# jzbontar/mc-cnn

Measured on AMD Instinct MI355X. Metric: Mega-pixel-disparities/sec (cost-vol+CBCA+SGM) + end-to-end disp ms/pair, higher is better.
Workload: dtype f32; 1 GPU; KITTI 2012 fast, 370x1226 disp_max=228; H=370, W=1226, disp_max=228, feature_channels=64, params=kitti_fast, parallelism=one pair per GPU

## Files before the change

mc-cnn_amd/csrc/post.hip:

```cpp
#include "launchers.h"

#include <atomic>

namespace mc {


__global__ void __launch_bounds__(256) fill_nan_kernel(float *__restrict__ p, int64_t n)
{
	const float nanv = __builtin_nanf("");
	for (int64_t i = (int64_t)blockIdx.x * blockDim.x + threadIdx.x; i < n; i += (int64_t)gridDim.x * blockDim.x) p[i] = nanv;
}

__global__ void __launch_bounds__(256) scale_kernel(const float *__restrict__ in, float *__restrict__ out, int64_t n, float s)
{
	for (int64_t i = (int64_t)blockIdx.x * blockDim.x + threadIdx.x; i < n; i += (int64_t)gridDim.x * blockDim.x) out[i] = in[i] * s;
}
typedef float f4v_t __attribute__((ext_vector_type(4)));
__global__ void __launch_bounds__(256) scale4_kernel(const f4v_t *__restrict__ in, f4v_t *__restrict__ out, int64_t n4, float s)
{
	const int64_t i = (int64_t)blockIdx.x * 256 + threadIdx.x;
	if (i < n4) out[i] = in[i] * s;
}

template <bool NT>
// ... 7 lines not shown
		const int64_t r = r0 + k, c = c0 + tx;
		if (r < R && c < Cn) tile[k][tx] = NT ? __builtin_nontemporal_load(in + r * ldin + c) : in[r * ldin + c];
	}
	__syncthreads();
	for (int k = ty; k < 64; k += 4) {
		const int64_t c = c0 + k, r = r0 + tx;
		if (r < R && c < Cn) {
			if (NT) __builtin_nontemporal_store(tile[tx][k] * s, out + c * ldout + r);
			else out[c * ldout + r] = tile[tx][k] * s;
		}
	}
}

typedef float post_f4 __attribute__((ext_vector_type(4)));
template <bool NT, bool LOOP_R>
__global__ void __launch_bounds__(256) transpose4_kernel(const float *__restrict__ in, float *__restrict__ out, int64_t R,
                                                         int64_t Cn, int64_t ldin, int64_t ldout, float s)
{
	__shared__ float tile[64][65];
	const int lx = threadIdx.x & 15, ly = threadIdx.x >> 4;
	const int64_t fixed0 = (int64_t)blockIdx.x * 64;
	const int64_t nloop = LOOP_R ? R : Cn;
	for (int64_t t0 = 0; t0 < nloop; t0 += 64) {
		const int64_t c0 = LOOP_R ? fixed0 : t0, r0 = LOOP_R ? t0 : fixed0;
#pragma unroll
		for (int k = 0; k < 4; ++k) {
			const int row = ly + 16 * k;
			const int64_t r = r0 + row, c = c0 + 4 * lx;
			if (r < R && c < Cn) {
				const post_f4 *p = (const post_f4 *)(in + r * ldin + c);
				const post_f4 v = NT ? __builtin_nontemporal_load(p) : *p;
				tile[row][4 * lx + 0] = v.x; tile[row][4 * lx + 1] = v.y; tile[row][4 * lx + 2] = v.z; tile[row][4 * lx + 3] = v.w;
			}
		}
		__syncthreads();
#pragma unroll
		for (int k = 0; k < 4; ++k) {
			const int col = ly + 16 * k;
			const int64_t c = c0 + col, r = r0 + 4 * lx;
			if (c < Cn && r < R) {
				const post_f4 v = {tile[4 * lx + 0][col] * s, tile[4 * lx + 1][col] * s, tile[4 * lx + 2][col] * s, tile[4 * lx + 3][col] * s};
				post_f4 *q = (post_f4 *)(out + c * ldout + r);
				if (NT) __builtin_nontemporal_store(v, q);
				else *q = v;
			}
		}
		__syncthreads();
	}
}


int fill_nan(float *p, int64_t n, hipStream_t st)
{
	if (n <= 0) return 0;
	const unsigned blocks = cdiv(n, 256) < 4096u ? cdiv(n, 256) : 4096u;
	hipLaunchKernelGGL(fill_nan_kernel, dim3(blocks), dim3(256), 0, st, p, n);
	return check_launch("fill_nan");
}

int scale(const float *in, float *out, int64_t n, float s, hipStream_t st)
{
	if (n <= 0) return 0;
	if (n % 4 == 0 && (uintptr_t)in % 16 == 0 && (uintptr_t)out % 16 == 0 && n / 4 / 256 < 0x7fffffff) {
		hipLaunchKernelGGL(scale4_kernel, dim3(cdiv(n / 4, 256)), dim3(256), 0, st, (const f4v_t *)in, (f4v_t *)out, n / 4, s);
		return check_launch("scale");
	}
	const unsigned blocks = cdiv(n, 256) < 4096u ? cdiv(n, 256) : 4096u;
	hipLaunchKernelGGL(scale_kernel, dim3(blocks), dim3(256), 0, st, in, out, n, s);
	return check_launch("scale");
}

int transpose(const float *in, float *out, int64_t R, int64_t Cn, int64_t ldin, int64_t ldout, float s, hipStream_t st, int nt)
{
	const bool use_nt = nt >= 0 ? nt != 0 : R * Cn * 4 > ((int64_t)768 << 20);
	const bool aligned16 = Cn % 4 == 0 && ldin % 4 == 0 && ldout % 4 == 0 && (uintptr_t)in % 16 == 0 && (uintptr_t)out % 16 == 0;
	if (R % 4 == 0 && aligned16) {
		if (R <= Cn) {
			if (use_nt) hipLaunchKernelGGL((transpose4_kernel<true, true>), dim3(cdiv(Cn, 64)), dim3(256), 0, st, in, out, R, Cn, ldin, ldout, s);
			else hipLaunchKernelGGL((transpose4_kernel<false, true>), dim3(cdiv(Cn, 64)), dim3(256), 0, st, in, out, R, Cn, ldin, ldout, s);
		} else {
			if (use_nt) hipLaunchKernelGGL((transpose4_kernel<true, false>), dim3(cdiv(R, 64)), dim3(256), 0, st, in, out, R, Cn, ldin, ldout, s);
			else hipLaunchKernelGGL((transpose4_kernel<false, false>), dim3(cdiv(R, 64)), dim3(256), 0, st, in, out, R, Cn, ldin, ldout, s);
		}
		return check_launch("transpose");
	}
	if (use_nt) hipLaunchKernelGGL(transpose_kernel<true>, dim3(cdiv(Cn, 64), cdiv(R, 64)), dim3(256), 0, st, in, out, R, Cn, ldin, ldout, s);
	else hipLaunchKernelGGL(transpose_kernel<false>, dim3(cdiv(Cn, 64), cdiv(R, 64)), dim3(256), 0, st, in, out, R, Cn, ldin, ldout, s);
	return check_launch("transpose");
}

__global__ void __launch_bounds__(256) fix_border_kernel(float *__restrict__ vol, int64_t rows, int W, int n, int direction)
{
	const int64_t id = (int64_t)blockIdx.x * blockDim.x + threadIdx.x;
	if (id >= rows * n) return;
	const int i = (int)(id % n) + 1;
	const int64_t r = id / n;
	const int dst = direction < 0 ? W - i : i - 1;
	const int src = direction < 0 ? W - (n + 1) : n;
	vol[r * W + dst] = vol[r * W + src];
}

int fix_border(float *vol, int D, int H, int W, int n, int direction, hipStream_t st)
{
	if (n <= 0) return 0;
	const int64_t rows = (int64_t)D * H;
	hipLaunchKernelGGL(fix_border_kernel, dim3(cdiv(rows * n, 256)), dim3(256), 0, st, vol, rows, W, n, direction);
	return check_launch("fix_border");
}

__global__ void __launch_bounds__(256) argmin_dhw_kernel(const float *__restrict__ vol, float *__restrict__ out, int D, int64_t HW,
                                                         int base1)
{
	const int64_t p = (int64_t)blockIdx.x * blockDim.x + threadIdx.x;
	if (p >= HW) return;
	int argmin = 0;
	float mn = __builtin_inff();
	for (int i = 0; i < D; ++i) {
		const float val = __builtin_nontemporal_load(vol + i * HW + p);
		if (val < mn) {
			mn = val;
			argmin = i;
		}
	}
	out[p] = (float)(argmin + base1);
}

__global__ void __launch_bounds__(256) argmin_dhw4_kernel(const float *__restrict__ vol, float *__restrict__ out, int D, int64_t HW,
                                                          int base1)
{
	const int64_t p = ((int64_t)blockIdx.x * blockDim.x + threadIdx.x) * 4;
	if (p >= HW) return;
	int a0 = 0, a1 = 0, a2 = 0, a3 = 0;
	float m0 = __builtin_inff(), m1 = m0, m2 = m0, m3 = m0;
	for (int i = 0; i < D; ++i) {
		const post_f4 v = __builtin_nontemporal_load((const post_f4 *)(vol + i * HW + p));
		if (v.x < m0) { m0 = v.x; a0 = i; }
		if (v.y < m1) { m1 = v.y; a1 = i; }
		if (v.z < m2) { m2 = v.z; a2 = i; }
		if (v.w < m3) { m3 = v.w; a3 = i; }
	}
	*(post_f4 *)(out + p) = post_f4{(float)(a0 + base1), (float)(a1 + base1), (float)(a2 + base1), (float)(a3 + base1)};
}

int argmin_dhw(const float *vol, float *out, int D, int H, int W, int base1, hipStream_t st)
{
	const int64_t HW = (int64_t)H * W;
	if (HW % 4 == 0 && (uintptr_t)vol % 16 == 0 && (uintptr_t)out % 16 == 0)
		hipLaunchKernelGGL(argmin_dhw4_kernel, dim3(cdiv(HW / 4, 256)), dim3(256), 0, st, vol, out, D, HW, base1);
	else
		hipLaunchKernelGGL(argmin_dhw_kernel, dim3(cdiv(HW, 256)), dim3(256), 0, st, vol, out, D, HW, base1);
	return check_launch("argmin_dhw");
}

__global__ void __launch_bounds__(256) outlier_rows_kernel(const float *__restrict__ d0, const float *__restrict__ d1,
                                                           float *__restrict__ outlier, int W, int disp_max)
{
	extern __shared__ unsigned char mark[];
	const int y = blockIdx.x;
	const int64_t row = (int64_t)y * W;
	for (int x = threadIdx.x; x < W; x += 256) mark[x] = 0;
	__syncthreads();
	for (int xp = threadIdx.x; xp < W; xp += 256) {
		const float v = d1[row + xp];
		if (v > -2.0f && v < (float)disp_max + 2.0f) {
			const int base = (int)floorf(v);
#pragma unroll
			for (int k = -2; k <= 3; ++k) {
				const int d = base + k;
				if (d >= 0 && d < disp_max && xp + d < W && (double)fabsf((float)d - v) < 1.1) mark[xp + d] = 1;
			}
		}
	}
	__syncthreads();
	for (int x = threadIdx.x; x < W; x += 256) {
		const int64_t id = row + x;
		const int d0i = (int)d0[id];
		float res;
		if (x - d0i < 0) res = 1;
		else if ((double)fabsf(d0[id] - d1[id - d0i]) < 1.1) res = 0;
		else res = mark[x] ? 2.0f : 1.0f;
		outlier[id] = res;
	}
}

struct LdsRaised {
	std::atomic<int> cus[64] = {};
	int raise(const void *kernel, int bytes, const char *who, int *ncu = nullptr)
	{
		int dev = 0;
		hipError_t e = hipGetDevice(&dev);
		if (e == hipSuccess && (dev < 0 || dev >= 64)) e = hipErrorInvalidDevice;
		if (e != hipSuccess) {
			set_error("%s: hipGetDevice: %s (device %d)", who, hipGetErrorString(e), dev);
			return (int)e;
		}
		int n = cus[dev].load(std::memory_order_acquire);
		if (!n) {
			e = hipFuncSetAttribute(kernel, hipFuncAttributeMaxDynamicSharedMemorySize, bytes);
			if (e == hipSuccess) e = hipDeviceGetAttribute(&n, hipDeviceAttributeMultiprocessorCount, dev);
			if (e != hipSuccess || n <= 0) {
				set_error("%s: %d bytes of dynamic LDS on device %d: %s", who, bytes, dev, hipGetErrorString(e));
				return e != hipSuccess ? (int)e : MC_EINVAL;
			}
			cus[dev].store(n, std::memory_order_release);
		}
		if (ncu) *ncu = n;
		return 0;
	}
};

int outlier_detection(const float *d0, const float *d1, float *outlier, int H, int W, int disp_max, hipStream_t st)
{
	MC_REQUIRE(W <= 160 * 1024, "outlier_detection: a row of %d pixels needs more than the 160 KiB of LDS its marks live in", W);
	if (W > 64 * 1024) {
		static LdsRaised raised;
		const int rc = raised.raise((const void *)outlier_rows_kernel, 160 * 1024, "outlier_detection");
		if (rc) return rc;
	}
	hipLaunchKernelGGL(outlier_rows_kernel, dim3(H), dim3(256), (size_t)W, st, d0, d1, outlier, W, disp_max);
	return check_launch("outlier_detection");
}

__global__ void __launch_bounds__(256) interp_occ_rows_kernel(const float *__restrict__ d0, const float *__restrict__ outlier,
                                                              float *__restrict__ out, int W, unsigned *__restrict__ mask, int size)
{
	__shared__ int carry[256];
	__shared__ int first_valid;
	const int y = blockIdx.x, t = threadIdx.x;
	const int64_t row = (int64_t)y * W;
	if (mask) {
		const int wa = (int)((row + 31) >> 5), wb = (int)((row + W + 31) >> 5);
		for (int w0 = wa; w0 < wb; w0 += 8) {
			const int p = w0 * 32 + t;
			const uint64_t bal = __ballot(p < size && outlier[p] == 2);
			const int w = w0 + (t >> 5);
			if ((t & 31) == 0 && w < wb) mask[w] = (unsigned)(bal >> (t & 32));
		}
	}
	const int seg = (W + 255) / 256;
	const int xa = t * seg, xb = min(W, xa + seg);
	if (t == 0) first_valid = W;
	int last = -1;
	for (int x = xa; x < xb; ++x)
		if (outlier[row + x] == 0) last = x;
	carry[t] = last;
	__syncthreads();
	if (last >= 0) {
		int f = -1;
		for (int x = xa; x < xb; ++x)
			if (outlier[row + x] == 0) { f = x; break; }
		atomicMin(&first_valid, f);
	}
	for (int off = 1; off < 256; off <<= 1) {
		const int o = t >= off ? carry[t - off] : -1;
		__syncthreads();
		carry[t] = max(carry[t], o);
		__syncthreads();
	}
	int lv = t > 0 ? carry[t - 1] : -1;
	const int fv = first_valid;
	for (int x = xa; x < xb; ++x) {
		const int64_t id = row + x;
		const float o = outlier[id];
		if (o == 0) lv = x;
		float r = d0[id];
		if (o == 1) {
			if (lv >= 0) r = d0[row + lv];
			else if (fv < W) r = d0[row + fv];
		}
		out[id] = r;
	}
}

int interpolate_occlusion(const float *d0, const float *outlier, float *out, int H, int W, hipStream_t st, unsigned *mask)
{
	if (mask) MC_REQUIRE((int64_t)H * W < ((int64_t)1 << 31), "interpolate_occlusion: %dx%d pixels do not fit the mask's 32-bit index", H, W);
	hipLaunchKernelGGL(interp_occ_rows_kernel, dim3(H), dim3(256), 0, st, d0, outlier, out, W, mask, mask ? H * W : 0);
	return check_launch("interpolate_occlusion");
}

template <int K> __device__ __forceinline__ void ray_rank_step(float v, int inb, int &less, int &eq)
{
	const float ov = __uint_as_float(__builtin_amdgcn_update_dpp(0u, __float_as_uint(v), 0x120 + K, 0xf, 0xf, false));
	const int oin = __builtin_amdgcn_update_dpp(0, inb, 0x120 + K, 0xf, 0xf, false);
	less += (oin && ov < v) ? 1 : 0;
	eq += (oin && ov == v) ? 1 : 0;
}

#define MC_MIS_NU 4
constexpr int MIS_NT = 1024;
constexpr unsigned MIS_OOB = 0x80000000u;

__device__ __forceinline__ void ray_select(float v, int inb, int ray, int id, const float *__restrict__ d0, float *__restrict__ out)
{
	int less = 0, eq = inb;
	ray_rank_step<1>(v, inb, less, eq); ray_rank_step<2>(v, inb, less, eq); ray_rank_step<3>(v, inb, less, eq);
	ray_rank_step<4>(v, inb, less, eq); ray_rank_step<5>(v, inb, less, eq); ray_rank_step<6>(v, inb, less, eq);
	ray_rank_step<7>(v, inb, less, eq); ray_rank_step<8>(v, inb, less, eq); ray_rank_step<9>(v, inb, less, eq);
	ray_rank_step<10>(v, inb, less, eq); ray_rank_step<11>(v, inb, less, eq); ray_rank_step<12>(v, inb, less, eq);
	ray_rank_step<13>(v, inb, less, eq); ray_rank_step<14>(v, inb, less, eq); ray_rank_step<15>(v, inb, less, eq);
	const uint64_t bal = __ballot(inb != 0);
	const int n = __builtin_popcount((unsigned)((bal >> ((threadIdx.x & 48))) & 0xffffu));
	if (n == 0) {
		if (ray == 0) out[id] = d0[id];
		return;
	}
	const int want = n / 2;
	if (inb && less <= want && want < less + eq) out[id] = v;
}

__device__ __forceinline__ void mis_rays_masked(const float *__restrict__ d0, const float *__restrict__ outlier, float *__restrict__ out,
                                                int size, int H, int W, const unsigned *__restrict__ mask, int per)
{
	static_assert(MC_MIS_NU == 4, "the round below is two whole-pixel steps");
	extern __shared__ unsigned mis_lds[];
	__shared__ int wave_n[MIS_NT / 64];
	__shared__ int next_item;
	const int nw = (size + 31) >> 5;
	unsigned *lmask = mis_lds;
	unsigned *slot = lmask + nw;
	int *list_y = (int *)(slot + MIS_NT * 16);
	unsigned short *list = (unsigned short *)(list_y + MIS_NT);
	const int tid = threadIdx.x, lane = tid & 63, wid = tid >> 6;
	const int pa = blockIdx.x * per, pb = min(size, pa + per);
	if (pa >= pb) return;
	for (int i = tid; i < nw; i += MIS_NT) lmask[i] = mask[i];
	constexpr unsigned HX_LO = 0x10000012u, HX_HI = 0x34444432u, HY_LO = 0x00123444u, HY_HI = 0x44321000u;
	const unsigned xmax2 = 2u * (unsigned)W - 2u, ymax2 = 2u * (unsigned)H - 2u;
	for (int c0 = pa; c0 < pb; c0 += MIS_NT) {
		const int p = c0 + tid;
		bool mis = false;
		if (p < pb) {
			const float v = d0[p];
			mis = outlier[p] == 2;
			if (!mis) out[p] = v;
		}
		const uint64_t bal = __ballot(mis);
		if (lane == 0) wave_n[wid] = __builtin_popcountll(bal);
		if (tid == 0) next_item = MIS_NT;
		__syncthreads();
		int base = 0, nlist = 0;
#pragma unroll
		for (int k = 0; k < MIS_NT / 64; ++k) {
			const int c = wave_n[k];
			base += k < wid ? c : 0;
			nlist += c;
		}
		if (mis) {
			const int j = base + __builtin_popcountll(bal & (((uint64_t)1 << lane) - 1));
			list[j] = (unsigned short)tid;
			list_y[j] = p / W;
		}
		__syncthreads();
		const int nitems = nlist * 16;
		int i = tid;
		int q = 0, X2 = 0, Y2 = 0, sx = 0, sy = 0, o1 = 0, o2 = 0;
		auto start = [&]() {
			const int j = i >> 4, ray = i & 15, sh = 4 * (ray & 7);
			sx = (int)(((ray < 8 ? HX_LO : HX_HI) >> sh) & 15u) - 2;
			sy = (int)(((ray < 8 ? HY_LO : HY_HI) >> sh) & 15u) - 2;
			q = c0 + list[j];
			const int y = list_y[j];
			X2 = 2 * (q - y * W);
			Y2 = 2 * y;
			o1 = ((sy + 1) >> 1) * W + ((sx + 1) >> 1);
			o2 = sy * W + sx;
		};
		if (i < nitems) start();
		while (i < nitems) {
			const int o[MC_MIS_NU] = {o1, o2, o2 + o1, 2 * o2};
			unsigned off[MC_MIS_NU], m[MC_MIS_NU];
#pragma unroll
			for (int k = 0; k < MC_MIS_NU; ++k) {
				X2 += sx;
				Y2 += sy;
				const bool in = (unsigned)X2 <= xmax2 && (unsigned)Y2 <= ymax2;
				const unsigned a = in ? (unsigned)(q + o[k]) : 0u;
				off[k] = in ? a : MIS_OOB;
				m[k] = lmask[a >> 5] >> (a & 31);
				m[k] = in ? m[k] & 1u : 0u;
			}
			q += 2 * o2;
			unsigned stop = MIS_OOB;
			bool stopped = false;
#pragma unroll
			for (int k = MC_MIS_NU - 1; k >= 0; --k) {
				const bool hit = m[k] == 0;
				stop = hit ? off[k] : stop;
				stopped = hit ? true : stopped;
			}
			if (stopped) {
				slot[i] = stop;
				i = atomicAdd(&next_item, 1);
				if (i < nitems) start();
			}
		}
		__syncthreads();
		const int ray = tid & 15;
		int j = tid >> 4;
		unsigned stop = j < nlist ? slot[j * 16 + ray] : MIS_OOB;
		float v = d0[stop != MIS_OOB ? stop : 0u];
		while (j < nlist) {
			const int jn = j + MIS_NT / 16;
			const unsigned stop_n = jn < nlist ? slot[jn * 16 + ray] : MIS_OOB;
			const float v_n = d0[stop_n != MIS_OOB ? stop_n : 0u];
			ray_select(stop != MIS_OOB ? v : 0.0f, stop != MIS_OOB ? 1 : 0, ray, c0 + list[j], d0, out);
			j = jn;
			stop = stop_n;
			v = v_n;
		}
		__syncthreads();
	}
}

__global__ void __launch_bounds__(MIS_NT) interp_mis_rays_kernel(const float *__restrict__ d0, const float *__restrict__ outlier,
                                                                 float *__restrict__ out, int size, int H, int W,
                                                                 const unsigned *__restrict__ mask, int per)
{
	if (mask) {
		mis_rays_masked(d0, outlier, out, size, H, W, mask, per);
		return;
	}
	const int t = blockIdx.x * blockDim.x + threadIdx.x;
// ... 404 lines not shown
```

mc-cnn_amd/csrc/sgm.hip:

```cpp
#include "launchers.h"

#define MC_SGM_VOL_AUX 2
#define MC_SGM_ST_AUX MC_SGM_VOL_AUX

namespace mc {

constexpr int SGM_PADW = 520;

struct SgmPassArgs {
	const float *C[2];
	const float *accin[2];
	const float *accin2[2];
	float *out[2];
	float *out2[2];
	float *disp[2];
	int drop_out[2];
	int direction[2];
	int nvol;
	int H, W, D, ds;
	int tri;
	const uint8_t *cls0;
	int64_t cls_plane;
	const uint8_t *win;
	int Wm;
	float P1[3], P2[3], P1a[3];
	int drop_h[2];
};

__device__ __forceinline__ int cls_of(float v, float tau) { return v < tau ? 0 : (v > tau ? 2 : 1); }

__global__ void __launch_bounds__(256) sgm_prep_kernel(const float *__restrict__ x0, const float *__restrict__ x1,
                                                       uint8_t *__restrict__ cls0, uint8_t *__restrict__ win,
                                                       int H, int W, int Wm, int64_t cls_plane, float tau_so)
{
	const int64_t id = (int64_t)blockIdx.x * blockDim.x + threadIdx.x;
	const int64_t total = (int64_t)4 * H * Wm;
	if (id >= total) return;
	const int i = (int)(id % Wm);
	const int y = (int)((id / Wm) % H);
	const int r = (int)(id / ((int64_t)Wm * H));
	const int dx = r == 0 ? 1 : (r == 1 ? -1 : 0);
	const int dy = r == 2 ? 1 : (r == 3 ? -1 : 0);
	const bool yok = (y - dy >= 0) && (y - dy < H);

	if (i < W) {
		const int x = i;
		int c = 1;
		if (yok && x - dx >= 0 && x - dx < W) {
			c = cls_of(fabsf(x0[y * W + x] - x0[(y - dy) * W + x - dx]), tau_so);
		}
		cls0[(int64_t)r * cls_plane + (int64_t)y * W + x] = (uint8_t)c;
	}
	const int s = i - SGM_PADW;
	unsigned asc = 0, desc = 0;
#pragma unroll
	for (int k = 0; k < 4; ++k) {
		const int xx = s + k;
		float D2 = 10.0f;
		if (yok && xx >= 0 && xx < W && xx - dx >= 0 && xx - dx < W) {
			D2 = fabsf(x1[y * W + xx] - x1[(y - dy) * W + xx - dx]);
		}
		const unsigned c = (unsigned)cls_of(D2, tau_so);
		asc |= c << (2 * k);
		desc |= c << (2 * (3 - k));
	}
	win[((int64_t)(0 * 4 + r) * H + y) * Wm + i] = (uint8_t)asc;
	win[((int64_t)(1 * 4 + r) * H + y) * Wm + i] = (uint8_t)desc;
}

typedef unsigned uint4v __attribute__((ext_vector_type(4)));

template <int VPL, int NACC>
struct StepData {
	float c[VPL];
	float a[NACC > 0 ? VPL : 1];
	float a2[NACC > 1 ? VPL : 1];
	unsigned pk;
	unsigned a0;
};


__device__ __forceinline__ float vmin2(float a, float b)
{
	float r;
	asm("v_min_f32 %0, %1, %2" : "=v"(r) : "v"(a), "v"(b));
	return r;
}
__device__ __forceinline__ float vmin3(float a, float b, float c)
{
	float r;
	asm("v_min3_f32 %0, %1, %2, %3" : "=v"(r) : "v"(a), "v"(b), "v"(c));
	return r;
}
__device__ __forceinline__ float wave_min_q(float v)
{
	float r;
	asm volatile("s_nop 1\n\tv_min_f32_dpp %1, %1, %1 quad_perm:[1,0,3,2] row_mask:0xf bank_mask:0xf\n\t"
	             "s_nop 1\n\tv_min_f32_dpp %1, %1, %1 quad_perm:[2,3,0,1] row_mask:0xf bank_mask:0xf\n\t"
	             "s_nop 1\n\tv_min_f32_dpp %1, %1, %1 row_half_mirror row_mask:0xf bank_mask:0xf\n\t"
	             "s_nop 1\n\tv_min_f32_dpp %1, %1, %1 row_mirror row_mask:0xf bank_mask:0xf\n\t"
	             "s_nop 1\n\tv_min_f32_dpp %1, %1, %1 row_bcast:15 row_mask:0xa bank_mask:0xf\n\t"
	             "s_nop 1\n\tv_min_f32_dpp %1, %1, %1 row_bcast:31 row_mask:0xc bank_mask:0xf\n\t"
	             "s_nop 0\n\tv_readlane_b32 %0, %1, 63"
	             : "=s"(r), "+v"(v));
	return r;
}

__device__ __forceinline__ __amdgpu_buffer_rsrc_t pixel_rsrc(const float *base, int64_t elem_off, int bytes)
{
	return __builtin_amdgcn_make_buffer_rsrc((void *)(base + elem_off), 0, bytes, 0x00020000);
}

template <int DIRN, int VPL, int MODE, bool ARGMIN, bool VEC, int U, bool DUAL, bool FAR, bool TRIH>
__device__ __forceinline__ void sgm_line(const SgmPassArgs &A, int wave)
{
	static_assert(!TRIH || (DIRN == 0 && DUAL && MODE == 0 && VEC && !FAR && !ARGMIN), "TRIH: the fused horizontal launch only");
	constexpr int NACC = MODE == 0 ? 0 : (MODE == 3 ? 2 : 1);
	const int lane = threadIdx.x & 63;
	const int H = A.H, W = A.W, D = A.D, ds = A.ds, Wm = A.Wm;
	const int nlines = DIRN <= 1 ? H : W;
	const int nsteps = DIRN <= 1 ? W : H;
	const int nw = A.nvol * nlines;
	bool second = false;
	if (DUAL) {
		if (wave >= 2 * nw) return;
		second = wave >= nw;
		if (second) wave -= nw;
	} else if (wave >= nw) {
		return;
	}
	const int dirn = (DUAL && second) ? 1 : DIRN;
	const int v = wave / nlines;
	const int line = wave - v * nlines;
	const int direction = A.direction[v];
	const float *__restrict__ Cp = A.C[v];
	const float *__restrict__ Ain = A.accin[v];
	const float *__restrict__ Ain2 = A.accin2[v];
	float *__restrict__ Out = (DUAL && second) ? A.out2[v] : A.out[v];
	float *__restrict__ Disp = A.disp[v];
	const bool drop = A.drop_out[v];

	const int x0s = dirn == 0 ? 0 : (dirn == 1 ? W - 1 : line);
	const int y0s = dirn == 2 ? 0 : (dirn == 3 ? H - 1 : line);
	const int sx = dirn == 0 ? 1 : (dirn == 1 ? -1 : 0);
	const int sy = dirn == 2 ? 1 : (dirn == 3 ? -1 : 0);

	const int dbase = VPL * lane;
	const uint8_t *__restrict__ cls0 = A.cls0 + (int64_t)dirn * A.cls_plane;
	constexpr int WBIAS = 1024;
	const uint8_t *__restrict__ win = A.win + ((int64_t)((direction > 0 ? 0 : 1) * 4 + dirn) * H) * Wm + SGM_PADW - WBIAS;
	const int woff = (direction > 0 ? dbase : -dbase - 3) + WBIAS;
	const int wq = direction > 0 ? 4 : -4;
	const int run_bytes = (VEC ? ds : D) * 4;
	constexpr bool TRI = DIRN >= 2 && MODE >= 2;
	int Dv = D;
	if (TRI && A.tri) Dv = __builtin_amdgcn_readfirstlane(min(D, direction < 0 ? line + 1 : W - line));
	const unsigned live_bytes = (TRI && Dv < D) ? (unsigned)Dv * 4u : (unsigned)run_bytes;

	const float INF = __builtin_inff();
	const float P1mid = A.P1[1], P2mid = A.P2[1], P1amid = A.P1a[1];
	const float P1lo = A.P1[0], P2lo = A.P2[0], P1alo = A.P1a[0];
	const float P1hi = A.P1[2], P2hi = A.P2[2], P1ahi = A.P1a[2];

	const int last = nsteps - 1;
	const int pix0 = y0s * W + x0s, dp = sy * W + sx;
	const int minpix = dp > 0 ? pix0 : pix0 + last * dp;
	const unsigned c1v = (unsigned)(dp * ds * 4);
	const unsigned c0v = dp > 0 ? 0u : (unsigned)last * (unsigned)(-dp * ds * 4);
	const unsigned span = (unsigned)last * (unsigned)((dp > 0 ? dp : -dp) * ds * 4) + (unsigned)run_bytes;
	constexpr unsigned OOBV = 0x80000000u;
	const __amdgpu_buffer_rsrc_t rC = pixel_rsrc(Cp, (int64_t)minpix * ds, FAR ? 0 : span);
	const __amdgpu_buffer_rsrc_t rA = pixel_rsrc(NACC >= 1 ? Ain : Cp, (int64_t)minpix * ds, FAR ? 0 : span);
	const __amdgpu_buffer_rsrc_t rA2 = pixel_rsrc(NACC >= 2 ? Ain2 : Cp, (int64_t)minpix * ds, FAR ? 0 : span);
	const __amdgpu_buffer_rsrc_t rO = pixel_rsrc(Out, (int64_t)minpix * ds, (FAR || drop) ? 0 : span);
	const __amdgpu_buffer_rsrc_t rW = __builtin_amdgcn_make_buffer_rsrc((void *)win, 0, H * Wm + 2 * WBIAS + 64, 0x00020000);
	const int w0 = y0s * Wm + x0s, dw = sy * Wm + sx;
	const __amdgpu_buffer_rsrc_t rCls = __builtin_amdgcn_make_buffer_rsrc((void *)cls0, 0, H * W, 0x00020000);
	const __amdgpu_buffer_rsrc_t rDisp = pixel_rsrc(ARGMIN ? Disp : Out, 0, H * W * 4);
	unsigned lane_off[VEC ? VPL / 4 : VPL];
#pragma unroll
	for (int q = 0; q < (VEC ? VPL / 4 : VPL); ++q) {
		const unsigned b = (unsigned)(dbase + (VEC ? 4 * q : q)) * 4u;
		lane_off[q] = ((FAR && !TRI) || b < live_bytes) ? b : OOBV;
	}
	const unsigned lane0_off = lane == 0 ? 0u : OOBV;
	const int hdv0 = direction < 0 ? x0s + 1 : W - x0s, hdv1 = direction < 0 ? sx : -sx;
	const bool trim_st = TRIH && (second || A.drop_h[v] != 0);
	const int sdv0 = trim_st ? hdv0 : D, sdv1 = trim_st ? hdv1 : 0;
	auto live_bytes_of = [&](int dv) -> unsigned { return dv < D ? (unsigned)dv * 4u : (unsigned)run_bytes; };
	auto live_at = [&](int s) -> unsigned { return live_bytes_of(hdv0 + s * hdv1); };
	auto piece_off = [&](int q, unsigned lim) -> unsigned {
		const unsigned b = (unsigned)(dbase + 4 * q) * 4u;
		return b < lim ? b : OOBV;
	};

	auto load_run = [&](float (&dst)[VPL], const float *base, const __amdgpu_buffer_rsrc_t &rs, unsigned so, int64_t pix, unsigned lim = 0u) {
		const __amdgpu_buffer_rsrc_t r = FAR ? pixel_rsrc(base, pix * ds, run_bytes) : rs;
		const unsigned soff = FAR ? 0u : so;
		if (VEC) {
#pragma unroll
			for (int q = 0; q < VPL / 4; ++q) {
				const uint4v t = __builtin_amdgcn_raw_buffer_load_b128(r, TRIH ? piece_off(q, lim) : lane_off[q], soff, MC_SGM_VOL_AUX);
				dst[4 * q + 0] = __uint_as_float(t.x); dst[4 * q + 1] = __uint_as_float(t.y);
				dst[4 * q + 2] = __uint_as_float(t.z); dst[4 * q + 3] = __uint_as_float(t.w);
			}
		} else {
#pragma unroll
			for (int j = 0; j < VPL; ++j) dst[j] = __uint_as_float(__builtin_amdgcn_raw_buffer_load_b32(r, lane_off[j], soff, 0));
		}
	};

	auto load_step = [&](StepData<VPL, NACC> &sd, int s) {
		const unsigned so = c0v + (unsigned)s * c1v;
		const int64_t pix = FAR ? (int64_t)(y0s + s * sy) * W + (x0s + s * sx) : 0;
		load_run(sd.c, Cp, rC, so, pix, TRIH ? live_at(s) : 0u);
		if constexpr (NACC >= 1) load_run(sd.a, Ain, rA, so, pix);
		if constexpr (NACC >= 2) load_run(sd.a2, Ain2, rA2, so, pix);
		unsigned pk = 0;
		const unsigned sw = (unsigned)(w0 + s * dw);
#pragma unroll
// ... 58 lines not shown
		}
		const int a0 = __builtin_amdgcn_readfirstlane((int)sd.a0);
		const int amatch = a0 == 1 ? 3 : a0;
		float P1x, P2x, P1ax = 0.0f;
		if (DIRN >= 2)
			asm("s_cmp_eq_u32 %3, 0\n\ts_cselect_b32 %0, %4, %5\n\ts_cselect_b32 %1, %6, %7\n\ts_cselect_b32 %2, %8, %9"
			    : "=s"(P1x), "=s"(P2x), "=s"(P1ax)
			    : "s"(a0), "s"(P1lo), "s"(P1hi), "s"(P2lo), "s"(P2hi), "s"(P1alo), "s"(P1ahi)
			    : "scc");
		else
			asm("s_cmp_eq_u32 %2, 0\n\ts_cselect_b32 %0, %3, %4\n\ts_cselect_b32 %1, %5, %6"
			    : "=s"(P1x), "=s"(P2x)
			    : "s"(a0), "s"(P1lo), "s"(P1hi), "s"(P2lo), "s"(P2hi)
			    : "scc");
		const float down = lane_from_below(prev[VPL - 1], INF);
		const float up = lane_from_above(prev[0], INF);
#pragma unroll
		for (int j = 0; j < VPL; ++j) {
			const int b = (sd.pk >> (2 * j)) & 3;
			const bool match = b == amatch;
			const float P2 = match ? P2x : P2midv;
			const float P1 = match ? P1x : P1midv;
			const float P1a = match ? P1ax : P1amidv;
			const float pm = j > 0 ? prev[j > 0 ? j - 1 : 0] : down;
			const float pp = j < VPL - 1 ? prev[j < VPL - 1 ? j + 1 : 0] : up;
			float cost;
			asm("v_min_f32 %0, %1, %2\n\tv_min3_f32 %0, %0, %3, %4"
			    : "=&v"(cost)
			    : "v"(prev[j]), "v"(m + P2), "v"(pm + (DIRN == 2 ? P1a : P1)), "v"(pp + (DIRN == 3 ? P1a : P1)));
			val[j] = (c[j] + cost) - m;
		}
		if (s == 0) {
			asm volatile("; border step");
#pragma unroll
			for (int j = 0; j < VPL; ++j) val[j] = c[j];
		}
		float q[VPL];
#pragma unroll
		for (int j = 0; j < VPL; ++j) {
			if (MODE == 0) o[j] = val[j] + zadd;
			else if (MODE == 1) o[j] = sd.a[j] + val[j];
			else if (MODE == 2) o[j] = (sd.a[j] + val[j]) * 0.25f;
			else o[j] = (sd.a[j] + sd.a2[j]) + val[j];
			q[j] = vmin2(val[j], INFv);
		}
#pragma unroll
		for (int j = 0; j < VPL; ++j) prev[j] = (dbase + j < Dv) ? q[j] : INFv;
		float nm = vmin3(prev[0], prev[1], prev[2]);
#pragma unroll
		for (int j = 3; j < VPL; j += 2) nm = j + 1 < VPL ? vmin3(nm, prev[j], prev[j + 1]) : vmin2(nm, prev[j]);
		m = wave_min_q(nm);
		if (keep) {
#pragma unroll
			for (int j = 0; j < VPL; ++j) keep[j] = o[j];
		} else {
			store_step(o, s);
		}
	};

	StepData<VPL, NACC> ring[U];
#pragma unroll
	for (int u = 0; u < U; ++u) load_step(ring[u], u < last ? u : last);

	int g = 0;
	constexpr int SB = (DIRN <= 1 && !ARGMIN && U % 4 == 0) ? 4 : 1;
	constexpr int LB = (DIRN <= 1 && U % 4 == 0) ? 4 : 1;
	float obuf[SB][VPL];
	for (; g + U <= nsteps; g += U) {
#pragma unroll
		for (int u = 0; u < U; ++u) {
			const int s = g + u;
			__builtin_amdgcn_sched_barrier(0);
			if (SB > 1) {
				process(ring[u], s, obuf[u % SB]);
				if (u % SB == SB - 1) {
#pragma unroll
					for (int k = 0; k < SB; ++k) store_step(obuf[k], s - (SB - 1) + k);
				}
			} else {
				process(ring[u], s);
			}
			if (u % LB == LB - 1) {
#pragma unroll
				for (int k = 0; k < LB; ++k) {
					const int sn = s - (LB - 1) + k + U;
					load_step(ring[u - (LB - 1) + k], sn < last ? sn : last);
				}
			}
		}
	}
#pragma unroll
	for (int u = 0; u < U; ++u) {
		if (g + u < nsteps) process(ring[u], g + u);
	}
}

template <int DIRN, int VPL, int MODE, bool ARGMIN, bool VEC, int U, bool DUAL, bool FAR>
__global__ void __launch_bounds__(256) sgm_pass_kernel(const SgmPassArgs A)
{
	const int wave = __builtin_amdgcn_readfirstlane((int)((blockIdx.x * blockDim.x + threadIdx.x) >> 6));
	if constexpr (DIRN == 0 && DUAL && MODE == 0 && VEC && !FAR && !ARGMIN) {
		if (A.tri) {
			sgm_line<DIRN, VPL, MODE, ARGMIN, VEC, U, DUAL, FAR, true>(A, wave);
			return;
		}
	}
	sgm_line<DIRN, VPL, MODE, ARGMIN, VEC, U, DUAL, FAR, false>(A, wave);
}


__global__ void __launch_bounds__(256) sgm_contract_kernel(const float *__restrict__ vol, int64_t pixels, int D, unsigned *__restrict__ count)
{
	const int64_t p = (int64_t)blockIdx.x * blockDim.x + threadIdx.x;
	bool bad = false;
	if (p < pixels) {
		const float *v = vol + p * D;
		bad = !(fabsf(v[0]) < __builtin_inff());
		bool seen_nan = false;
		for (int d = 0; d < D; ++d) {
			const bool isn = v[d] != v[d];
			bad = bad || (seen_nan && !isn);
			seen_nan = seen_nan || isn;
		}
	}
	const unsigned long long b = __ballot(bad);
	if ((threadIdx.x & 63) == 0 && b) atomicAdd(count, (unsigned)__builtin_popcountll(b));
}

int sgm_contract_violations(const float *vol, int H, int W, int D, unsigned *count, hipStream_t st)
{
	const int64_t pixels = (int64_t)H * W;
	hipError_t e = hipMemsetAsync(count, 0, sizeof(unsigned), st);
	if (e != hipSuccess) {
		set_error("mc_sgm2_contract_violations: hipMemsetAsync: %s", hipGetErrorString(e));
		return (int)e;
	}
	hipLaunchKernelGGL(sgm_contract_kernel, dim3(cdiv(pixels, 256)), dim3(256), 0, st, vol, pixels, D, count);
	return check_launch("sgm_contract");
}

struct SgmMaps { int Wm; size_t plane, cls0, win, bytes; };
static SgmMaps sgm_maps(int H, int W)
{
	const int Wm = W + 2 * SGM_PADW;
	const size_t plane = ((size_t)H * W + 3 + 4) / 4 * 4;
	return {Wm, plane, 0, 4 * plane, (4 * plane + (size_t)8 * H * Wm + 255) & ~(size_t)255};
}

size_t sgm_maps_bytes(int H, int W) { return sgm_maps(H, W).bytes; }

int sgm_prep(const float *x0, const float *x1, void *maps, int H, int W, float tau_so, hipStream_t st)
{
	const SgmMaps m = sgm_maps(H, W);
	const int64_t total = (int64_t)4 * H * m.Wm;
	hipLaunchKernelGGL(sgm_prep_kernel, dim3(cdiv(total, 256)), dim3(256), 0, st, x0, x1, (uint8_t *)maps + m.cls0, (uint8_t *)maps + m.win, H, W,
	                   m.Wm, (int64_t)m.plane, tau_so);
	return check_launch("sgm_prep");
}

constexpr int SGM_U_H = 8, SGM_U_UP = 16;
constexpr int SGM_U_DOWN = 16;

template <int DIRN, int MODE, bool ARGMIN, bool DUAL>
static void launch_pass(const SgmPassArgs &A, bool vec, hipStream_t st)
{
	const int nlines = DIRN <= 1 ? A.H : A.W;
	const int waves = A.nvol * nlines * (DUAL ? 2 : 1);
	const dim3 grid(cdiv(waves, 4)), block(256);
	const int U = DIRN == 2 ? SGM_U_DOWN : (DIRN == 3 ? SGM_U_UP : SGM_U_H);
	constexpr bool SCALAR = MODE == 1;
#define MC_SGM_GO(VPL_, VEC_, U_) \
	hipLaunchKernelGGL((sgm_pass_kernel<DIRN, VPL_, MODE, ARGMIN, VEC_, U_, DUAL, false>), grid, block, 0, st, A)
#define MC_SGM_GO_FAR(VPL_, VEC_, U_) \
	hipLaunchKernelGGL((sgm_pass_kernel<DIRN, VPL_, MODE, ARGMIN, VEC_, U_, DUAL, true>), grid, block, 0, st, A)
	const bool far = (int64_t)A.H * A.W * A.ds * 4 >= ((int64_t)1 << 31);
	if (!vec) {
		if constexpr (SCALAR) {
			if (far) { if (A.D <= 256) MC_SGM_GO_FAR(4, false, 4); else MC_SGM_GO_FAR(8, false, 2); }
			else { if (A.D <= 256) MC_SGM_GO(4, false, 4); else MC_SGM_GO(8, false, 2); }
		}
	} else if (far) {
		if (A.D <= 256) MC_SGM_GO_FAR(4, true, 4); else MC_SGM_GO_FAR(8, true, 4);
	} else if (A.D <= 256) {
		if (U == 16) MC_SGM_GO(4, true, 16); else if (U == 8) MC_SGM_GO(4, true, 8); else MC_SGM_GO(4, true, 4);
	} else {
		if (U >= 8) MC_SGM_GO(8, true, 8); else MC_SGM_GO(8, true, 4);
	}
#undef MC_SGM_GO_FAR
#undef MC_SGM_GO
}


int sgm_sweeps(const float *const C[2], float *const out[2], float *const out2[2], float *const disp[2],
               const int direction[2], int nvol, int H, int W, int D, int ds, const void *maps, float pi1, float pi2,
               float alpha1, float q1, float q2, bool fused, unsigned drop_final, bool tri, hipStream_t st)
{
	MC_REQUIRE((int64_t)H * W < ((int64_t)1 << 29) && (int64_t)W * ds * 4 < ((int64_t)1 << 31), "sgm: image %dx%d (pixel stride %d) exceeds the sweeps' 32-bit line arithmetic", H, W, ds);
	SgmPassArgs A;
	for (int v = 0; v < 2; ++v) {
		const int k = v < nvol ? v : 0;
		A.C[v] = C[k];
		A.accin[v] = out[k];
		A.accin2[v] = out2 ? out2[k] : nullptr;
		A.out[v] = out[k];
		A.out2[v] = out2 ? out2[k] : nullptr;
		A.disp[v] = disp ? disp[k] : nullptr;
		A.direction[v] = direction[k];
		A.drop_out[v] = 0;
		A.drop_h[v] = (fused && tri && v < nvol && ((drop_final >> v) & 1)) ? 1 : 0;
	}
	A.nvol = nvol;
	A.tri = (fused && tri) ? 1 : 0;
	A.H = H; A.W = W; A.D = D; A.ds = ds;
	const SgmMaps m = sgm_maps(H, W);
	A.Wm = m.Wm;
	A.cls0 = (const uint8_t *)maps + m.cls0;
	A.cls_plane = (int64_t)m.plane;
	A.win = (const uint8_t *)maps + m.win;
	A.P1[0] = pi1; A.P2[0] = pi2;
	A.P1[1] = pi1 / q1; A.P2[1] = pi2 / q1;
	A.P1[2] = pi1 / (q1 * q2); A.P2[2] = pi2 / (q1 * q2);
	for (int k = 0; k < 3; ++k) A.P1a[k] = A.P1[k] / alpha1;

	bool vec = (ds % 4 == 0);
	for (int v = 0; v < nvol; ++v) {
		vec = vec && ((uintptr_t)C[v] % 16 == 0) && ((uintptr_t)out[v] % 16 == 0);
		if (out2) vec = vec && ((uintptr_t)out2[v] % 16 == 0);
	}
	const bool am = fused && disp && disp[0];
	if (!fused) {
		launch_pass<0, 1, false, false>(A, vec, st);
		launch_pass<1, 1, false, false>(A, vec, st);
		launch_pass<2, 1, false, false>(A, vec, st);
		launch_pass<3, 1, false, false>(A, vec, st);
	} else {
		MC_REQUIRE(out2 && vec, "sgm: the fused sweeps need the second direction's scratch and 16-byte aligned volumes with ds %% 4 == 0");
		launch_pass<0, 0, false, true>(A, vec, st);
		launch_pass<2, 3, false, false>(A, vec, st);
		for (int v = 0; v < nvol; ++v) A.drop_out[v] = (drop_final >> v) & 1;
		if (am) launch_pass<3, 2, true, false>(A, vec, st);
		else launch_pass<3, 2, false, false>(A, vec, st);
	}
	return check_launch("sgm_pass");
}

}
```

Measured before the change: 86370 MPix-disp/s.

## Restructure post-processing and SGM prep kernels for register reuse and vector stores

outlier_rows_kernel now preloads up to eight d0/d1 values per thread into registers and reuses them for both the scatter and classify phases, instead of re-reading them from global memory. interp_occ_rows_kernel keeps its per-thread segment in registers and replaces the 256-wide LDS scan with barriers by a wave shuffle scan plus a small per-wave combine. sgm_prep_kernel computes each class once into LDS and writes 4-byte packed stores, instead of recomputing four neighbours per byte and storing single bytes. The cost is extra register pressure and more complex edge and alignment handling. These are small post-processing and prep kernels, so the effect on the end-to-end metric is likely limited.

Result: no change. 86830 MPix-disp/s, median of 6 (+0.5%).

```diff
diff --git a/mc-cnn_amd/csrc/post.hip b/mc-cnn_amd/csrc/post.hip
--- a/mc-cnn_amd/csrc/post.hip
+++ b/mc-cnn_amd/csrc/post.hip
@@ -183,16 +183,33 @@
 	return check_launch("argmin_dhw");
 }
 
+constexpr int OUT_R = 8;
 __global__ void __launch_bounds__(256) outlier_rows_kernel(const float *__restrict__ d0, const float *__restrict__ d1,
                                                            float *__restrict__ outlier, int W, int disp_max)
 {
 	extern __shared__ unsigned char mark[];
 	const int y = blockIdx.x;
 	const int64_t row = (int64_t)y * W;
+	float a0[OUT_R], a1[OUT_R], am[OUT_R];
+#pragma unroll
+	for (int j = 0; j < OUT_R; ++j) {
+		const int x = threadIdx.x + 256 * j;
+		a0[j] = x < W ? d0[row + x] : 0.0f;
+	}
+#pragma unroll
+	for (int j = 0; j < OUT_R; ++j) {
+		const int x = threadIdx.x + 256 * j;
+		a1[j] = x < W ? d1[row + x] : 0.0f;
+	}
+#pragma unroll
+	for (int j = 0; j < OUT_R; ++j) {
+		const int x = threadIdx.x + 256 * j;
+		const int d0i = (int)a0[j];
+		am[j] = (x < W && x - d0i >= 0) ? d1[row + x - d0i] : 0.0f;
+	}
 	for (int x = threadIdx.x; x < W; x += 256) mark[x] = 0;
 	__syncthreads();
-	for (int xp = threadIdx.x; xp < W; xp += 256) {
-		const float v = d1[row + xp];
+	auto scatter = [&](int xp, float v) {
 		if (v > -2.0f && v < (float)disp_max + 2.0f) {
 			const int base = (int)floorf(v);
 #pragma unroll
@@ -201,16 +218,27 @@
 				if (d >= 0 && d < disp_max && xp + d < W && (double)fabsf((float)d - v) < 1.1) mark[xp + d] = 1;
 			}
 		}
-	}
+	};
+#pragma unroll
+	for (int j = 0; j < OUT_R; ++j)
+		if (threadIdx.x + 256 * j < W) scatter(threadIdx.x + 256 * j, a1[j]);
+	for (int xp = threadIdx.x + 256 * OUT_R; xp < W; xp += 256) scatter(xp, d1[row + xp]);
 	__syncthreads();
-	for (int x = threadIdx.x; x < W; x += 256) {
-		const int64_t id = row + x;
-		const int d0i = (int)d0[id];
+	auto classify = [&](int x, float v0, float vm) {
+		const int d0i = (int)v0;
 		float res;
 		if (x - d0i < 0) res = 1;
-		else if ((double)fabsf(d0[id] - d1[id - d0i]) < 1.1) res = 0;
+		else if ((double)fabsf(v0 - vm) < 1.1) res = 0;
 		else res = mark[x] ? 2.0f : 1.0f;
-		outlier[id] = res;
+		outlier[row + x] = res;
+	};
+#pragma unroll
+	for (int j = 0; j < OUT_R; ++j)
+		if (threadIdx.x + 256 * j < W) classify(threadIdx.x + 256 * j, a0[j], am[j]);
+	for (int x = threadIdx.x + 256 * OUT_R; x < W; x += 256) {
+		const float v0 = d0[row + x];
+		const int d0i = (int)v0;
+		classify(x, v0, x - d0i >= 0 ? d1[row + x - d0i] : 0.0f);
 	}
 }
 
@@ -252,13 +280,24 @@
 	return check_launch("outlier_detection");
 }
 
+constexpr int OCC_R = 8;
 __global__ void __launch_bounds__(256) interp_occ_rows_kernel(const float *__restrict__ d0, const float *__restrict__ outlier,
                                                               float *__restrict__ out, int W, unsigned *__restrict__ mask, int size)
 {
-	__shared__ int carry[256];
-	__shared__ int first_valid;
-	const int y = blockIdx.x, t = threadIdx.x;
+	__shared__ int wave_last[4], wave_first[4];
+	const int y = blockIdx.x, t = threadIdx.x, lane = t & 63, wid = t >> 6;
 	const int64_t row = (int64_t)y * W;
+	const int seg = (W + 255) / 256;
+	const int xa = min(W, t * seg), xb = min(W, xa + seg);
+	const bool inreg = seg <= OCC_R;
+	float oc[OCC_R], dv[OCC_R];
+	if (inreg) {
+#pragma unroll
+		for (int j = 0; j < OCC_R; ++j) {
+			oc[j] = xa + j < xb ? outlier[row + xa + j] : -1.0f;
+			dv[j] = xa + j < xb ? d0[row + xa + j] : 0.0f;
+		}
+	}
 	if (mask) {
 		const int wa = (int)((row + 31) >> 5), wb = (int)((row + W + 31) >> 5);
 		for (int w0 = wa; w0 < wb; w0 += 8) {
@@ -268,38 +307,54 @@
 			if ((t & 31) == 0 && w < wb) mask[w] = (unsigned)(bal >> (t & 32));
 		}
 	}
-	const int seg = (W + 255) / 256;
-	const int xa = t * seg, xb = min(W, xa + seg);
-	if (t == 0) first_valid = W;
-	int last = -1;
-	for (int x = xa; x < xb; ++x)
-		if (outlier[row + x] == 0) last = x;
-	carry[t] = last;
+	int last = -1, first = W;
+	if (inreg) {
+#pragma unroll
+		for (int j = 0; j < OCC_R; ++j)
+			if (oc[j] == 0) {
+				last = xa + j;
+				first = min(first, xa + j);
+			}
+	} else {
+		for (int x = xa; x < xb; ++x)
+			if (outlier[row + x] == 0) {
+				last = x;
+				first = min(first, x);
+			}
+	}
+	int inc = last;
+#pragma unroll
+	for (int off = 1; off < 64; off <<= 1) {
+		const int o = __shfl_up(inc, off);
+		if (lane >= off) inc = max(inc, o);
+	}
+	const int before = __shfl_up(inc, 1);
+	const uint64_t any = __ballot(last >= 0);
+	const int wfirst = __shfl(first, any ? __ffsll((unsigned long long)any) - 1 : 0);
+	if (lane == 63) wave_last[wid] = inc;
+	if (lane == 0) wave_first[wid] = wfirst;
 	__syncthreads();
-	if (last >= 0) {
-		int f = -1;
-		for (int x = xa; x < xb; ++x)
-			if (outlier[row + x] == 0) { f = x; break; }
-		atomicMin(&first_valid, f);
-	}
-	for (int off = 1; off < 256; off <<= 1) {
-		const int o = t >= off ? carry[t - off] : -1;
-		__syncthreads();
-		carry[t] = max(carry[t], o);
-		__syncthreads();
-	}
-	int lv = t > 0 ? carry[t - 1] : -1;
-	const int fv = first_valid;
-	for (int x = xa; x < xb; ++x) {
-		const int64_t id = row + x;
-		const float o = outlier[id];
+	int lv = lane > 0 ? before : -1;
+	int fv = W;
+#pragma unroll
+	for (int w = 0; w < 4; ++w) {
+		if (w < wid) lv = max(lv, wave_last[w]);
+		fv = min(fv, wave_first[w]);
+	}
+	auto fill = [&](int x, float o, float r) {
 		if (o == 0) lv = x;
-		float r = d0[id];
 		if (o == 1) {
 			if (lv >= 0) r = d0[row + lv];
 			else if (fv < W) r = d0[row + fv];
 		}
-		out[id] = r;
+		out[row + x] = r;
+	};
+	if (inreg) {
+#pragma unroll
+		for (int j = 0; j < OCC_R; ++j)
+			if (xa + j < xb) fill(xa + j, oc[j], dv[j]);
+	} else {
+		for (int x = xa; x < xb; ++x) fill(x, outlier[row + x], d0[row + x]);
 	}
 }
 
diff --git a/mc-cnn_amd/csrc/sgm.hip b/mc-cnn_amd/csrc/sgm.hip
--- a/mc-cnn_amd/csrc/sgm.hip
+++ b/mc-cnn_amd/csrc/sgm.hip
@@ -29,43 +29,83 @@
 
 __device__ __forceinline__ int cls_of(float v, float tau) { return v < tau ? 0 : (v > tau ? 2 : 1); }
 
-__global__ void __launch_bounds__(256) sgm_prep_kernel(const float *__restrict__ x0, const float *__restrict__ x1,
-                                                       uint8_t *__restrict__ cls0, uint8_t *__restrict__ win,
-                                                       int H, int W, int Wm, int64_t cls_plane, float tau_so)
-{
-	const int64_t id = (int64_t)blockIdx.x * blockDim.x + threadIdx.x;
-	const int64_t total = (int64_t)4 * H * Wm;
-	if (id >= total) return;
-	const int i = (int)(id % Wm);
-	const int y = (int)((id / Wm) % H);
-	const int r = (int)(id / ((int64_t)Wm * H));
+constexpr int SGM_PREP_NT = 64, SGM_PREP_COLS = 4 * SGM_PREP_NT;
+__host__ __device__ constexpr int sgm_prep_blocks(int Wm) { return (Wm + 3 + SGM_PREP_COLS - 1) / SGM_PREP_COLS; }
+
+__device__ __forceinline__ void sgm_prep_store(uint8_t *__restrict__ row, int i0, int n, uint32_t v)
+{
+	if (i0 >= 0 && i0 + 4 <= n) {
+		*reinterpret_cast<uint32_t *>(row + i0) = v;
+	} else {
+#pragma unroll
+		for (int j = 0; j < 4; ++j)
+			if (i0 + j >= 0 && i0 + j < n) row[i0 + j] = (uint8_t)(v >> (8 * j));
+	}
+}
+
+__device__ __forceinline__ unsigned sgm_prep_class(const float *__restrict__ img, int W, int y, int yb, int dx, bool ok, int x, float tau,
+                                                   unsigned outside)
+{
+	const float a = img[(int64_t)y * W + min(max(x, 0), W - 1)];
+	const float b = img[(int64_t)yb * W + min(max(x - dx, 0), W - 1)];
+	return (ok && x >= 0 && x < W && x - dx >= 0 && x - dx < W) ? (unsigned)cls_of(fabsf(a - b), tau) : outside;
+}
+
+__global__ void __launch_bounds__(SGM_PREP_NT) sgm_prep_kernel(const float *__restrict__ x0, const float *__restrict__ x1,
+                                                               uint8_t *__restrict__ cls0, uint8_t *__restrict__ win,
+                                                               int H, int W, int Wm, int64_t cls_plane, float tau_so)
+{
+	__shared__ uint32_t cls_ref[SGM_PREP_NT];
+	__shared__ uint32_t cls_par[SGM_PREP_NT + 1];
+	uint8_t *ref8 = reinterpret_cast<uint8_t *>(cls_ref), *par8 = reinterpret_cast<uint8_t *>(cls_par);
+	const int t = threadIdx.x;
+	const int bpr = sgm_prep_blocks(Wm);
+	const int kb = (int)(blockIdx.x % bpr);
+	const int y = (int)((blockIdx.x / bpr) % H);
+	const int r = (int)(blockIdx.x / ((unsigned)bpr * H));
 	const int dx = r == 0 ? 1 : (r == 1 ? -1 : 0);
 	const int dy = r == 2 ? 1 : (r == 3 ? -1 : 0);
 	const bool yok = (y - dy >= 0) && (y - dy < H);
-
-	if (i < W) {
-		const int x = i;
-		int c = 1;
-		if (yok && x - dx >= 0 && x - dx < W) {
-			c = cls_of(fabsf(x0[y * W + x] - x0[(y - dy) * W + x - dx]), tau_so);
-		}
-		cls0[(int64_t)r * cls_plane + (int64_t)y * W + x] = (uint8_t)c;
-	}
-	const int s = i - SGM_PADW;
-	unsigned asc = 0, desc = 0;
+	const int yb = yok ? y - dy : y;
+
+	uint8_t *c0 = cls0 + (int64_t)r * cls_plane + (int64_t)y * W;
+	const int xs0 = kb * SGM_PREP_COLS - (int)((uintptr_t)c0 & 3);
+	uint8_t *wa = win + ((int64_t)(0 * 4 + r) * H + y) * Wm;
+	uint8_t *wd = win + ((int64_t)(1 * 4 + r) * H + y) * Wm;
+	const int i00 = kb * SGM_PREP_COLS - (int)((uintptr_t)wa & 3);
+	const int s00 = i00 - SGM_PADW;
+	const unsigned cpad = (unsigned)cls_of(10.0f, tau_so);
+	const bool any_ref = xs0 < W;
+	const bool any_par = yok && s00 + SGM_PREP_COLS + 2 >= 0 && s00 < W;
+
+	if (any_ref) {
+#pragma unroll
+		for (int q = 0; q < 4; ++q) {
+			const int p = t + q * SGM_PREP_NT;
+			ref8[p] = (uint8_t)sgm_prep_class(x0, W, y, yb, dx, yok, xs0 + p, tau_so, 1u);
+		}
+	}
+	if (any_par) {
+#pragma unroll
+		for (int q = 0; q < 5; ++q) {
+			const int p = t + q * SGM_PREP_NT;
+			const unsigned c = sgm_prep_class(x1, W, y, yb, dx, true, s00 + p, tau_so, cpad);
+			if (p < SGM_PREP_COLS + 4) par8[p] = (uint8_t)c;
+		}
+	}
+	__syncthreads();
+
+	if (any_ref) sgm_prep_store(c0, xs0 + 4 * t, W, cls_ref[t]);
+	const uint64_t w = any_par ? (uint64_t)cls_par[t] | (uint64_t)cls_par[t + 1] << 32 : (uint64_t)cpad * 0x0101010101010101ull;
+	uint32_t asc = 0, desc = 0;
 #pragma unroll
 	for (int k = 0; k < 4; ++k) {
-		const int xx = s + k;
-		float D2 = 10.0f;
-		if (yok && xx >= 0 && xx < W && xx - dx >= 0 && xx - dx < W) {
-			D2 = fabsf(x1[y * W + xx] - x1[(y - dy) * W + xx - dx]);
-		}
-		const unsigned c = (unsigned)cls_of(D2, tau_so);
-		asc |= c << (2 * k);
-		desc |= c << (2 * (3 - k));
-	}
-	win[((int64_t)(0 * 4 + r) * H + y) * Wm + i] = (uint8_t)asc;
-	win[((int64_t)(1 * 4 + r) * H + y) * Wm + i] = (uint8_t)desc;
+		const uint32_t ck = (uint32_t)(w >> (8 * k));
+		asc |= ck << (2 * k);
+		desc |= ck << (2 * (3 - k));
+	}
+	sgm_prep_store(wa, i00 + 4 * t, Wm, asc);
+	sgm_prep_store(wd, i00 + 4 * t, Wm, desc);
 }
 
 typedef unsigned uint4v __attribute__((ext_vector_type(4)));
@@ -430,8 +470,9 @@
 int sgm_prep(const float *x0, const float *x1, void *maps, int H, int W, float tau_so, hipStream_t st)
 {
 	const SgmMaps m = sgm_maps(H, W);
-	const int64_t total = (int64_t)4 * H * m.Wm;
-	hipLaunchKernelGGL(sgm_prep_kernel, dim3(cdiv(total, 256)), dim3(256), 0, st, x0, x1, (uint8_t *)maps + m.cls0, (uint8_t *)maps + m.win, H, W,
+	const int64_t blocks = (int64_t)4 * H * sgm_prep_blocks(m.Wm);
+	MC_REQUIRE(blocks < ((int64_t)1 << 31), "sgm_prep: %dx%d needs more blocks than a grid has", H, W);
+	hipLaunchKernelGGL(sgm_prep_kernel, dim3((unsigned)blocks), dim3(SGM_PREP_NT), 0, st, x0, x1, (uint8_t *)maps + m.cls0, (uint8_t *)maps + m.win, H, W,
 	                   m.Wm, (int64_t)m.plane, tau_so);
 	return check_launch("sgm_prep");
 }
```
